# abmoRobotics/isaac_rover_orbit

Hardware: AMD Instinct MI355X
Metric: env-steps/sec AAURoverEnv-v0 @ num_envs=4096; 1/2/4/8 MI355X (higher is better)
Workload: dtype f32

## Files before the change

isaac_rover_orbit_amd/csrc/rover_diag.inc:

```
#pragma once
#if defined(RV_K1_STAMP) || defined(RV_K1_LITE)
__device__ unsigned long long *g_k1_stamps;
#endif
#ifdef RV_K1_LITE
__device__ __forceinline__ void k1_lite(int slot)
{
    if ((threadIdx.x & 255) == 0) {
        unsigned long long t;
        asm volatile("s_memtime %0\n\ts_waitcnt lgkmcnt(0)" : "=s"(t)::"memory");
        g_k1_stamps[(size_t)blockIdx.x * 64 + (threadIdx.x >> 8) * 32 + slot] = t;
    }
}
#define K1_LITE(k) k1_lite(k)
#endif
#ifdef RV_K1_LITE_FINE
#define K1_LITE_F(k) k1_lite(k)
#endif
#ifdef RV_K1_STAMP
__device__ __forceinline__ void k1_stamp(int slot)
{
    if (threadIdx.x == 0) {
        unsigned long long t;
        asm volatile("s_waitcnt vmcnt(0) lgkmcnt(0)\n\ts_memtime %0\n\ts_waitcnt lgkmcnt(0)" : "=s"(t)::"memory");
        g_k1_stamps[(size_t)blockIdx.x * 32 + slot] = t;
    }
}
#define K1_STAMP(k) k1_stamp(k)
#endif
```

isaac_rover_orbit_amd/csrc/rover_kernels.hip:

```cpp
#include <hip/hip_runtime.h>
#include <vector>

#include <cmath>
#include <cstdio>
#include <cstring>
#include <new>
#include <type_traits>

#include <dlfcn.h>

#include "../../include/rover_hip.h"
#include "../../include/rover_debug.h"
#include "rover_model.hpp"
#include "rover_internal.hpp"

namespace {

struct StepConsts {
    float h, inv_h, inv_m, inv_I[3];
    float steer_hkp, steer_den_inv, steer_i_over_h, steer_dv_max;
    float wheel_den_inv, wheel_h_over_i, lt_motor;
    float bogie_keep[3], b_winv[3];
    float bogie_gq[3];
};
__host__ __device__ inline void make_step_consts(float h, StepConsts &k)
{
    constexpr float INERTIA_B[3] = RV_INERTIA_B_INIT;
    constexpr float BOGIE_INERTIA[3] = RV_BOGIE_INERTIA_INIT;
    constexpr float SUBTREE_MASS[3] = RV_SUBTREE_MASS_INIT;
    k.h = h;
    k.inv_h = 1.0f / h;
    k.inv_m = 1.0f / RV_M_TOTAL;
    for (int i = 0; i < 3; ++i) k.inv_I[i] = 1.0f / INERTIA_B[i];
    k.steer_hkp = h * RV_STEER_KP;
    k.steer_den_inv = 1.0f / (RV_STEER_INERTIA + h * RV_STEER_KD + h * h * RV_STEER_KP);
    k.steer_i_over_h = RV_STEER_INERTIA / h;
    k.steer_dv_max = RV_STEER_EFFORT * h / RV_STEER_INERTIA;
    k.wheel_den_inv = 1.0f / (RV_WHEEL_INERTIA + h * RV_WHEEL_KD + h * h * RV_WHEEL_KP);
    k.wheel_h_over_i = h / RV_WHEEL_INERTIA;
    k.lt_motor = RV_WHEEL_EFFORT * h / RV_WHEEL_CONTACT_RADIUS;
    for (int j = 0; j < 3; ++j) {
        k.bogie_keep[j] = 1.0f / (1.0f + h * RV_BOGIE_DAMPING / BOGIE_INERTIA[j]);
        k.b_winv[j] = 1.0f / BOGIE_INERTIA[j];
        k.bogie_gq[j] = (-(SUBTREE_MASS[j] * RV_GRAVITY) * h) * k.b_winv[j];
    }
}

struct RvParams {
    rover_config cfg;
    StepConsts K;
    const float *height;
    const float *lookup;
    const float *obstacle;
    const uint8_t *safe_mask;
    const float *spawns;
    int H, W, n_spawns;
    float res, min_x, min_y;
    int n, env_id_offset;
    uint32_t spawn_a, spawn_b;
    int rays, obs_w;
    int tile_dim;
    int tile_pitch;
    const int16_t *height_q;
    float q_scale;
    int chunk_cells;
    float *scan_desc;
    float inv_res, x_max, y_max, inv_nx;
    int cpr_log;
    int wq, pq;
    int tile_bufs;
    uint32_t step_tag;
    unsigned *log_counter;
    int xcd_rows;
    int nt_obs;
};

__device__ __forceinline__ float clampf(float x, float lo, float hi) { return x < lo ? lo : (x > hi ? hi : x); }
__device__ __forceinline__ float clamp_med3(float x, float lo, float hi) { return __builtin_amdgcn_fmed3f(x, lo, hi); }
__device__ __forceinline__ float dot3(const float *a, const float *b) { return a[0] * b[0] + a[1] * b[1] + a[2] * b[2]; }
__device__ __forceinline__ void cross3(const float *a, const float *b, float *o)
{
    o[0] = a[1] * b[2] - a[2] * b[1];
    o[1] = a[2] * b[0] - a[0] * b[2];
    o[2] = a[0] * b[1] - a[1] * b[0];
}
__device__ __forceinline__ float sign_torch(float x) { return (float)((x > 0.0f) - (x < 0.0f)); }
__device__ __forceinline__ void quat_to_mat(const float *q, float R[3][3])
{
    const float w = q[0], x = q[1], y = q[2], z = q[3];
    R[0][0] = 1.0f - 2.0f * (y * y + z * z);
    R[0][1] = 2.0f * (x * y - w * z);
    R[0][2] = 2.0f * (x * z + w * y);
    R[1][0] = 2.0f * (x * y + w * z);
    R[1][1] = 1.0f - 2.0f * (x * x + z * z);
    R[1][2] = 2.0f * (y * z - w * x);
    R[2][0] = 2.0f * (x * z - w * y);
    R[2][1] = 2.0f * (y * z + w * x);
    R[2][2] = 1.0f - 2.0f * (x * x + y * y);
}
__device__ __forceinline__ void mat_vec(const float R[3][3], const float *v, float *o)
{
    o[0] = R[0][0] * v[0] + R[0][1] * v[1] + R[0][2] * v[2];
    o[1] = R[1][0] * v[0] + R[1][1] * v[1] + R[1][2] * v[2];
    o[2] = R[2][0] * v[0] + R[2][1] * v[1] + R[2][2] * v[2];
}

__device__ __forceinline__ void mat_tvec(const float R[3][3], const float *v, float *o)
{
    o[0] = R[0][0] * v[0] + R[1][0] * v[1] + R[2][0] * v[2];
    o[1] = R[0][1] * v[0] + R[1][1] * v[1] + R[2][1] * v[2];
    o[2] = R[0][2] * v[0] + R[1][2] * v[1] + R[2][2] * v[2];
}
__device__ __forceinline__ float wdot3x(const float *a, const float *b, const float *w) { return a[0] * b[0] * w[0] + a[1] * b[1] * w[1] + a[2] * b[2] * w[2]; }
__device__ __forceinline__ float wdot3(const float *a, const float *w) { return a[0] * a[0] * w[0] + a[1] * a[1] * w[1] + a[2] * a[2] * w[2]; }


__device__ __forceinline__ void rv_sincosf(float x, float *s, float *c)
{
    const float k = floorf(x * 0.63661977236758134f + 0.5f);
    float r = x - k * 1.5703125f;
    r = r - k * 4.837512969970703125e-4f;
    r = r - k * 7.54978995489188e-8f;
    const int q = ((int)k) & 3;
    const float z = r * r;
    const float sp = r + r * z * (-1.6666654611e-1f + z * (8.3321608736e-3f + z * (-1.9515295891e-4f)));
    const float cp = 1.0f - 0.5f * z + z * z * (4.166664568298827e-2f + z * (-1.388731625493765e-3f + z * 2.443315711809948e-5f));
    const float ss = (q & 1) ? cp : sp;
// ... 773 lines not shown
            link_body_forces(lf3[i], Fb);
#pragma unroll
            for (int b = 0; b < 7; ++b) F[b * 3 + i] = Fb[b];
        }
    }
    chassis_integrate(h, R, v, w, com_w, S + ROVER_POS, S + ROVER_QUAT, S + ROVER_LINVEL, S + ROVER_ANGVEL);
#pragma unroll
    for (int j = 0; j < 3; ++j) bogie_integrate(h, bq[j], bd[j], S[ROVER_BOGIE_Q + j], S[ROVER_BOGIE_QD + j]);
}

struct GroupLane {
    float pos[3], quat[4], linvel[3], angvel[3];
    float R[3][3], com_off[3];
    float bq, bqd, sq, sqd, wq, wqd, lam;
    float steer_t, wheel_t;
    float P[3], ax[3], b_winv, bogie_keep;
    float bogie_gq;
    SubConsts sub;
    float lp[3];
    ArmConsts arm;
    f2 minv0, minv1;
    bool steerable, wheel_active, role_b;
};

__device__ __forceinline__ float dpp_ror8(float x) { return __int_as_float(__builtin_amdgcn_update_dpp(0, __float_as_int(x), 0x128, 0xF, 0xF, true)); }
__device__ __forceinline__ void cross_role_sum3(float &a, float &b, float &c)
{
    asm volatile(
        "s_nop 1\n\t"
        "v_add_f32_dpp %0, %0, %0 row_ror:8 row_mask:0xf bank_mask:0xf bound_ctrl:1\n\t"
        "v_add_f32_dpp %1, %1, %1 row_ror:8 row_mask:0xf bank_mask:0xf bound_ctrl:1\n\t"
        "v_add_f32_dpp %2, %2, %2 row_ror:8 row_mask:0xf bank_mask:0xf bound_ctrl:1"
        : "+v"(a), "+v"(b), "+v"(c));
}
__device__ __forceinline__ void slot_sum4(float &a0, float &a1, float &a2, float &a3)
{
    asm volatile(
        "s_nop 1\n\t"
        "v_add_f32_dpp %0, %0, %0 quad_perm:[1,0,3,2] row_mask:0xf bank_mask:0xf bound_ctrl:1\n\t"
        "v_add_f32_dpp %1, %1, %1 quad_perm:[1,0,3,2] row_mask:0xf bank_mask:0xf bound_ctrl:1\n\t"
        "v_add_f32_dpp %2, %2, %2 quad_perm:[1,0,3,2] row_mask:0xf bank_mask:0xf bound_ctrl:1\n\t"
        "v_add_f32_dpp %3, %3, %3 quad_perm:[1,0,3,2] row_mask:0xf bank_mask:0xf bound_ctrl:1\n\t"
        "v_add_f32_dpp %0, %0, %0 quad_perm:[2,3,0,1] row_mask:0xf bank_mask:0xf bound_ctrl:1\n\t"
        "v_add_f32_dpp %1, %1, %1 quad_perm:[2,3,0,1] row_mask:0xf bank_mask:0xf bound_ctrl:1\n\t"
        "v_add_f32_dpp %2, %2, %2 quad_perm:[2,3,0,1] row_mask:0xf bank_mask:0x3 bound_ctrl:1\n\t"
        "v_add_f32_dpp %3, %3, %3 quad_perm:[2,3,0,1] row_mask:0xf bank_mask:0x3 bound_ctrl:1\n\t"
        "v_add_f32_dpp %0, %0, %0 row_half_mirror row_mask:0xf bank_mask:0xf bound_ctrl:1\n\t"
        "v_add_f32_dpp %1, %1, %1 row_half_mirror row_mask:0xf bank_mask:0xf bound_ctrl:1\n\t"
        "v_add_f32_dpp %2, %2, %2 row_half_mirror row_mask:0xf bank_mask:0x3 bound_ctrl:1\n\t"
        "v_add_f32_dpp %3, %3, %3 row_half_mirror row_mask:0xf bank_mask:0x3 bound_ctrl:1"
        : "+v"(a0), "+v"(a1), "+v"(a2), "+v"(a3));
}

#if defined(RV_K1_STAMP) || defined(RV_K1_LITE)
#include "rover_diag.inc"
#endif
#ifndef K1_STAMP
#define K1_STAMP(k) do { } while (0)
#endif
#ifndef K1_LITE
#define K1_LITE(k) do { } while (0)
#endif
#ifndef K1_LITE_F
#define K1_LITE_F(k) do { } while (0)
#endif
__device__ __forceinline__ void solver_iteration_generic(const StepConsts &K, Contact &ct, const RoleRows &rr, f2 *V, float mu)
{
    float un, ut, us;
    role_partials(rr, V, un, ut, us);
    cross_role_sum3(un, ut, us);
    float dn, dt, ds;
    impulse_update(K, ct, mu, un, ut, us, dn, dt, ds);
    f2 o[2];
    role_outputs(rr, dn, dt, ds, o);
    float a0 = o[0].x, a1 = o[0].y, a2 = o[1].x, a3 = o[1].y;
    slot_sum4(a0, a1, a2, a3);
    V[0] += (f2){a0, a1};
    V[1] += (f2){a2, a3};
}

#define RV_DPP_FULL " row_mask:0xf bank_mask:0xf bound_ctrl:1\n\t"
#define RV_DPP_LANES_A " row_mask:0xf bank_mask:0x3 bound_ctrl:1\n\t"
#define RV_BC_LO " op_sel_hi:[1,0,1]\n\t"
#define RV_BC_HI " op_sel:[0,1,0] op_sel_hi:[1,1,1]\n\t"
#define RV_SOLVER_HALF(LN_IN, LN_OUT, LT_IN, LT_OUT, LS_IN, LS_OUT, FILLER)                                            \
    "v_pk_fma_f32 v[240:241], %[jn0], %[v0], %[cn]\n\t"                                                              \
    "v_pk_fma_f32 v[242:243], %[jts0], %[v0], %[cts]" RV_BC_LO                                                       \
    "v_pk_fma_f32 v[240:241], %[jn1], %[v1], v[240:241]\n\t"                                                         \
    "v_pk_fma_f32 v[242:243], %[jts1], %[v0], v[242:243]" RV_BC_HI                                                   \
    "v_add_f32 v240, v240, v241\n\t"                      \
    "v_pk_fma_f32 v[242:243], %[jts2], %[v1], v[242:243]" RV_BC_LO                                                   \
    "v_pk_fma_f32 v[242:243], %[jts3], %[v1], v[242:243]" RV_BC_HI                                                   \
    "v_add_f32_dpp v240, v240, v240 row_ror:8" RV_DPP_FULL    \
    "v_fma_f32 v245, -v240, %[mn], " LN_IN "\n\t"                                                                    \
    "v_add_f32_dpp v242, v242, v242 row_ror:8" RV_DPP_FULL    \
    "v_add_f32_dpp v243, v243, v243 row_ror:8" RV_DPP_FULL    \
    "v_max_f32 " LN_OUT ", 0, v245\n\t"                     \
    "v_sub_f32 v246, " LN_OUT ", " LN_IN "\n\t"             \
    "v_mul_f32 v245, %[mu], " LN_OUT "\n\t"                 \
    "v_pk_mul_f32 v[252:253], %[mn0], v[246:247] op_sel_hi:[1,0]\n\t"                                                \
    "v_fmac_f32 v242, %[ant], v246\n\t"                     \
    "v_pk_mul_f32 v[254:255], %[mn1], v[246:247] op_sel_hi:[1,0]\n\t"                                                \
    "v_min_f32 v247, %[ltm], v245\n\t"                      \
    "v_fmac_f32 v243, %[ans], v246\n\t"                     \
    "v_fma_f32 v244, -v242, %[mt], " LT_IN "\n\t"                                                                    \
    "v_med3_f32 " LT_OUT ", v244, -v247, v247\n\t"          \
    "v_sub_f32 v248, " LT_OUT ", " LT_IN "\n\t"             \
    "v_fmac_f32 v243, %[ats], v248\n\t"                     \
    "v_pk_fma_f32 v[252:253], %[mt0], v[248:249], v[252:253] op_sel_hi:[1,0,1]\n\t"                                  \
    "v_fma_f32 v244, -v243, %[ms], " LS_IN "\n\t"                                                                    \
    "v_pk_fma_f32 v[254:255], %[mt1], v[248:249], v[254:255] op_sel_hi:[1,0,1]\n\t"                                  \
    "v_med3_f32 " LS_OUT ", v244, -v245, v245\n\t"          \
    "v_sub_f32 v250, " LS_OUT ", " LS_IN "\n\t"             \
    "v_pk_fma_f32 v[252:253], %[ms0], v[250:251], v[252:253] op_sel_hi:[1,0,1]\n\t"                                  \
    "v_pk_fma_f32 v[254:255], %[ms1], v[250:251], v[254:255] op_sel_hi:[1,0,1]\n\t"                                  \
    FILLER                                                                                                             \
    "v_add_f32_dpp v252, v252, v252 quad_perm:[1,0,3,2]" RV_DPP_FULL                                                   \
// ... 257 lines not shown
{
    const float cbx = S[ROVER_CMD_B], cby = S[ROVER_CMD_B + 1];
    float *o = obs + (size_t)e * p.obs_w;
    o[0] = S[ROVER_ACTION];
    o[1] = S[ROVER_ACTION + 1];
    o[2] = sqrtf(cbx * cbx + cby * cby) * p.cfg.obs_scale_distance;
    o[3] = rv_atan2f(cby, cbx) * p.cfg.obs_scale_heading;
}

struct ScanWindow {
    float px, py, pz, cy, sy;
    int i_lo, j_lo, th, tw4;
    int interior;
};
__device__ __forceinline__ ScanWindow scan_window(const RvParams &p, const float *pos, const float *quat)
{
    const rover_config &c = p.cfg;
    ScanWindow w;
    const float qw = quat[0], qx = quat[1], qy = quat[2], qz = quat[3];
    const float a = 1.0f - 2.0f * (qy * qy + qz * qz);
    const float b = 2.0f * (qw * qz + qx * qy);
    const float inv = 1.0f / sqrtf(a * a + b * b);
    w.px = pos[0]; w.py = pos[1]; w.pz = pos[2];
    w.cy = a * inv;
    w.sy = b * inv;
    const float inv_res = p.inv_res;
    const float hx = 0.5f * c.scan_size_x, hy = 0.5f * c.scan_size_y;
    const float ex = fabsf(w.cy) * hx + fabsf(w.sy) * hy, ey = fabsf(w.sy) * hx + fabsf(w.cy) * hy;
    int j_lo = (int)floorf((w.px - ex - p.min_x) * inv_res) - 1;
    int i_lo = (int)floorf((w.py - ey - p.min_y) * inv_res) - 1;
    int j_hi = (int)floorf((w.px + ex - p.min_x) * inv_res) + 2;
    int i_hi = (int)floorf((w.py + ey - p.min_y) * inv_res) + 2;
    j_lo = max(0, min(j_lo, p.W - 1)); j_hi = max(0, min(j_hi, p.W - 1));
    i_lo = max(0, min(i_lo, p.H - 1)); i_hi = max(0, min(i_hi, p.H - 1));
    const int cc = p.chunk_cells, sh = (cc == 8) ? 3 : 2;
    j_lo &= ~(cc - 1);
    w.i_lo = i_lo;
    w.j_lo = j_lo;
    w.th = min(i_hi - i_lo + 1, p.tile_dim);
    w.tw4 = min(min((j_hi - j_lo + cc) >> sh, p.tile_pitch >> sh), (p.W - j_lo + cc - 1) >> sh);
    const float m = 2.0f * p.res;
    w.interior = (w.px - ex > p.min_x + m) && (w.px + ex < p.x_max - m) && (w.py - ey > p.min_y + m) &&
                 (w.py + ey < p.y_max - m) && (i_hi - i_lo + 1 <= p.tile_dim) && (((j_hi - j_lo + cc) >> sh) <= (p.tile_pitch >> sh));
    return w;
}
__device__ __forceinline__ void write_scan_desc(const RvParams &p, const float *pos, const float *quat, int e)
{
    const ScanWindow w = scan_window(p, pos, quat);
    float4 *d = reinterpret_cast<float4 *>(p.scan_desc + (size_t)e * 8);
    d[0] = make_float4(w.px, w.py, w.pz, w.cy);
    d[1] = make_float4(w.sy, __int_as_float(w.i_lo), __int_as_float(w.j_lo), __int_as_float(w.th | (w.interior << 15) | (w.tw4 << 16)));
}

__device__ __forceinline__ float wave_sum(float x)
{
#pragma unroll
    for (int m = 32; m >= 1; m >>= 1) x += __shfl_xor(x, m, 64);
    return x;
}

template <int PHASE>
__device__ __forceinline__ void step_lane_body(const RvParams &p, float *__restrict__ state, const float *__restrict__ action,
                                               float *__restrict__ obs, float *__restrict__ reward, uint8_t *__restrict__ terminated,
                                               uint8_t *__restrict__ truncated, float *__restrict__ force, float *__restrict__ log_partial,
                                               const uint8_t *__restrict__ reset_mask)
{
    const int e_raw = blockIdx.x * 64 + threadIdx.x;
    const bool active = e_raw < p.n;
    const int e = active ? e_raw : p.n - 1;
    const int N = p.n;
    const rover_config &c = p.cfg;

    float S[ROVER_STATE_WORDS];
    float F[ROVER_NUM_BODIES * 3];
    if (PHASE == 2) {
#pragma unroll
        for (int i = 0; i < ROVER_STATE_WORDS; ++i) S[i] = state[(size_t)i * N + e];
#pragma unroll
        for (int i = 0; i < ROVER_NUM_BODIES * 3; ++i) F[i] = force[(size_t)i * N + e];
    } else {
#pragma unroll
        for (int i = 0; i < ROVER_TARGET_W; ++i) S[i] = state[(size_t)i * N + e];
#pragma unroll
        for (int i = ROVER_ACTION; i < ROVER_ACTION + 2; ++i) S[i] = state[(size_t)i * N + e];
#pragma unroll
        for (int i = ROVER_LAMBDA_N; i < ROVER_LAMBDA_N + 6; ++i) S[i] = state[(size_t)i * N + e];

        S[ROVER_PREV_ACTION] = S[ROVER_ACTION];
        S[ROVER_PREV_ACTION + 1] = S[ROVER_ACTION + 1];
        const float2 a = reinterpret_cast<const float2 *>(action)[e];
        S[ROVER_ACTION] = a.x;
        S[ROVER_ACTION + 1] = a.y;
        float steer_m[4], wheel_m[6];
        {
            float processed[2], steer[4], wheel[6];
            ackermann_one(c, S + ROVER_ACTION, processed, steer, wheel);
            steer_m[0] = steer[0]; steer_m[1] = steer[3]; steer_m[2] = steer[1]; steer_m[3] = steer[2];
            wheel_m[0] = wheel[1]; wheel_m[1] = wheel[5]; wheel_m[2] = wheel[0];
            wheel_m[3] = wheel[4]; wheel_m[4] = wheel[2]; wheel_m[5] = wheel[3];
        }

        const StepConsts &K = p.K;
        for (int s = 0; s < c.decimation - 1; ++s) physics_substep<false>(p, K, S, steer_m, wheel_m, nullptr);
        if (c.decimation > 0) {
            physics_substep<true>(p, K, S, steer_m, wheel_m, F);
        } else {
// ... 552 lines not shown
                const int r = private_ray_index(m, lane);
                if (r < p.rays) row[r] = o;
            }
        }
    }
}

template <bool TRI>
__device__ __forceinline__ void scan_single_tile_wave(const RvParams &p, int16_t *tile, int lane, int n_env, int e_base,
                                                      const PrivateWindows &w, float *__restrict__ out, int row_stride, int col0,
                                                      const float2 *__restrict__ ray_xy)
{
    if (n_env <= 0) return;
    private_issue(p, w, 0, tile, lane);
    f2 oxy[PRIVATE_ROUNDS];
#pragma unroll
    for (int m = 0; m < PRIVATE_ROUNDS; ++m) {
        const float2 v = ray_xy[m * 64 + lane];
        oxy[m] = (f2){v.x, v.y};
    }
#pragma unroll
    for (int j = 0; j < 4; ++j) {
        if (j < n_env) {
            asm volatile("s_waitcnt vmcnt(0)" ::: "memory");
            __builtin_amdgcn_wave_barrier();
            private_cast<TRI>(p, w, j, tile, lane, e_base, out, row_stride, col0, oxy, ray_xy);
            if (j + 1 < n_env) {
                asm volatile("s_waitcnt lgkmcnt(0)" ::: "memory");
                private_issue(p, w, j + 1, tile, lane);
            }
        }
    }
}

__device__ __forceinline__ void windows_to_lds(float *win, const ScanWindow &sw, int lane)
{
    if ((lane & 15) == 0) {
        float4 *d = reinterpret_cast<float4 *>(win + (lane >> 4) * 8);
        d[0] = make_float4(sw.px, sw.py, sw.pz, sw.cy);
        d[1] = make_float4(sw.sy, __int_as_float(sw.i_lo), __int_as_float(sw.j_lo), __int_as_float(sw.th | (sw.interior << 15) | (sw.tw4 << 16)));
    }
}
__device__ __forceinline__ void windows_from_lds(const float *win, PrivateWindows &w)
{
#pragma unroll
    for (int j = 0; j < 4; ++j) {
        const float4 d0 = reinterpret_cast<const float4 *>(win + j * 8)[0], d1 = reinterpret_cast<const float4 *>(win + j * 8)[1];
        auto uni = [](float v) { return __int_as_float(__builtin_amdgcn_readfirstlane(__float_as_int(v))); };
        w.px[j] = uni(d0.x); w.py[j] = uni(d0.y); w.pz[j] = uni(d0.z); w.cy[j] = uni(d0.w); w.sy[j] = uni(d1.x);
        w.i_lo[j] = __builtin_amdgcn_readfirstlane(__float_as_int(d1.y)); w.j_lo[j] = __builtin_amdgcn_readfirstlane(__float_as_int(d1.z));
        w.pk[j] = __builtin_amdgcn_readfirstlane(__float_as_int(d1.w));
    }
}
constexpr int RV_HAND = 448;
__device__ __forceinline__ float *fused_win(float *lds, const RvParams &p, int wv)
{
    return reinterpret_cast<float *>(reinterpret_cast<int16_t *>(lds) + (size_t)8 * p.tile_dim * p.tile_pitch) + wv * 64;
}
__device__ __forceinline__ float *fused_link(float *lds, const RvParams &p, int wv) { return fused_win(lds, p, 0) + 256 + wv * RV_HAND; }
template <bool TRI>
__device__ __forceinline__ void scan_copy_wave(const RvParams &p, const float *__restrict__ state, float *lds, int partner, int lane,
                                               float *__restrict__ obs, const float2 *__restrict__ ray_xy)
{
    const int tile_cells = p.tile_dim * p.tile_pitch;
    int16_t *tile0 = reinterpret_cast<int16_t *>(lds) + (size_t)(2 * partner) * tile_cells, *tile1 = tile0 + tile_cells;
    const float *win = fused_win(lds, p, partner);
    const int e_base = (int)(blockIdx.x * 4 + partner) * 4;
    const int n_env = max(0, min(4, p.n - e_base));
    PrivateWindows w;
    f2 oxy[PRIVATE_ROUNDS];
#pragma unroll
    for (int m = 0; m < PRIVATE_ROUNDS; ++m) {
        const float2 v = ray_xy[m * 64 + lane];
        oxy[m] = (f2){v.x, v.y};
    }
    {
        const int e = min(e_base + (lane >> 4), p.n - 1);
        const uint32_t count = __float_as_uint(state[(size_t)ROVER_RESET_COUNT * p.n + e]);
        ResetOutcome ro;
        reset_draw(p, (uint32_t)(p.env_id_offset + e), count, nullptr, ro);
        if ((lane & 15) == 0) {
            float4 *d = reinterpret_cast<float4 *>(fused_link(lds, p, partner) + 256 + (lane >> 4) * 12);
            d[0] = make_float4(ro.px, ro.py, ro.pz, ro.qw);
            d[1] = make_float4(ro.qz, ro.tx, ro.ty, ro.tz);
            d[2] = make_float4(ro.heading_cmd, 0.0f, 0.0f, 0.0f);
        }
    }
    {
        __syncthreads();
        const float *lk = fused_link(lds, p, partner);
        const SlotConst sc = d_SLOT[lane & 7];
        const bool role_b = (lane & 8) != 0;
        const float *pe = lk + (lane >> 4) * 12;
        const float R[3][3] = {{pe[0], pe[1], pe[2]}, {pe[3], pe[4], pe[5]}, {pe[6], pe[7], pe[8]}};
        const float pos[3] = {pe[9], pe[10], pe[11]};
        const float P[3] = {sc.P[0], sc.P[1], sc.P[2]}, ax[3] = {sc.ax[0], sc.ax[1], sc.ax[2]};
        float lp[3];
#pragma unroll
        for (int i = 0; i < 3; ++i) lp[i] = role_b ? sc.lp[1][i] : sc.lp[0][i];
        const float bq = lk[64 + lane];
        float bsc[2];
        bogie_sincos(bq, &bsc[0], &bsc[1]);
        const LinkSample ls = link_point_fetch(p, R, pos, P, ax, bq, lp, bsc);
        const float wbp[3] = {sc.wb[0], sc.wb[1], sc.wb[2]};
        const LinkSample ws = link_point_fetch(p, R, pos, P, ax, bq, wbp, bsc);
        float f3[3];
        link_point_eval(ls, p.inv_res, f3);
        const_cast<float *>(lk)[320 + lane] = f3[0];
        const_cast<float *>(lk)[384 + lane] = f3[1];
        const_cast<float *>(lk)[128 + lane] = f3[2];
        const_cast<float *>(lk)[192 + lane] = link_sample_obstacle(ws);
    }
    K1_LITE(0);
    __syncthreads();
    K1_LITE(1);
    {
        float *lk = const_cast<float *>(fused_link(lds, p, partner));
        const float4 d = reinterpret_cast<const float4 *>(lk + 48 + (lane >> 4) * 4)[0];
        const float4 q = reinterpret_cast<const float4 *>(lk + 304 + (lane >> 4) * 4)[0];
        const float pf[3] = {d.x, d.y, d.z}, qf[4] = {q.x, q.y, q.z, q.w};
        const ScanWindow sw = scan_window(p, pf, qf);
        private_windows(sw, w);
        if (n_env > 0) private_issue(p, w, 0, tile0, lane);
        float flag = 0.0f;
        for (int spin = 0; spin < (1 << 20); ++spin) {
            flag = *(volatile __attribute__((address_space(3))) float *)(__attribute__((address_space(3))) float *)(lk + 48 + (lane >> 4) * 4 + 3);
            if (__builtin_amdgcn_ballot_w64(flag == 0.0f) == 0ull) break;
            __builtin_amdgcn_s_sleep(1);
        }
        K1_LITE(2);
        const bool resets = flag == 2.0f;
        const unsigned long long rmask = __builtin_amdgcn_ballot_w64(resets);
        if (__builtin_expect(rmask != 0ull, 0)) {
            float pr[3] = {pf[0], pf[1], pf[2]}, qr[4] = {qf[0], qf[1], qf[2], qf[3]};
            if (resets) {
                const float4 *o = reinterpret_cast<const float4 *>(lk + 256 + (lane >> 4) * 12);
                const float4 o0 = o[0], o1 = o[1];
                pr[0] = o0.x; pr[1] = o0.y; pr[2] = o0.z;
                qr[0] = o0.w; qr[1] = 0.0f; qr[2] = 0.0f; qr[3] = o1.x;
            }
            const ScanWindow swr = scan_window(p, pr, qr);
            private_windows(swr, w);
            uniform_windows(w);
            windows_to_lds(const_cast<float *>(win), swr, lane);
            if (n_env > 0 && (rmask & 0x1ull)) { asm volatile("s_waitcnt vmcnt(0)" ::: "memory"); private_issue(p, w, 0, tile0, lane); }
        } else {
            windows_to_lds(const_cast<float *>(win), sw, lane);
        }
        if ((lane & 15) == 0)
            *(volatile __attribute__((address_space(3))) float *)(__attribute__((address_space(3))) float *)(lk + 48 + (lane >> 4) * 4 + 3) = 3.0f;
    }
    K1_LITE(3);
    asm volatile("s_waitcnt vmcnt(0)" ::: "memory");
    K1_LITE(4);
    if (n_env > 0) private_cast<TRI>(p, w, 0, tile0, lane, e_base, obs, p.obs_w, 4, oxy, ray_xy);
    K1_LITE(5);
    asm volatile("s_waitcnt lgkmcnt(0)" ::: "memory");
    K1_LITE(6);
    K1_LITE(7);
    if (n_env > 2) private_issue(p, w, 2, tile0, lane);
    K1_LITE(8);
    asm volatile("s_waitcnt vmcnt(0)" ::: "memory");
    K1_LITE(9);
    K1_LITE(10);
    K1_LITE(11);
    if (n_env > 2) private_cast<TRI>(p, w, 2, tile0, lane, e_base, obs, p.obs_w, 4, oxy, ray_xy);
    K1_LITE(12);
    K1_LITE(13);
    K1_LITE(14);
    K1_LITE(15);
}

enum StepForm { TWO_LAUNCH, COPY_WAVES, SINGLE_TILE };
template <StepForm FORM, bool TRI, bool BEGIN_ONLY = false>
__device__ __forceinline__ void step_group_body(const RvParams &p, float *__restrict__ state, const float *__restrict__ action,
                                                float *__restrict__ obs, float *__restrict__ reward, uint8_t *__restrict__ terminated,
                                                uint8_t *__restrict__ truncated, float *__restrict__ force,
                                                float *__restrict__ log_partial, float *lds, const float2 *__restrict__ ray_xy)
{
    const int lane = threadIdx.x & 63;
    const int wave = blockIdx.x * (RV_K1G_THREADS / 64) + (threadIdx.x >> 6);
    const int e_raw = wave * 4 + (lane >> 4);
    const bool active = e_raw < p.n;
    const int e = active ? e_raw : p.n - 1;
    const int N = p.n;
    const rover_config &c = p.cfg;
    const SlotConst sc = d_SLOT[lane & 7];
    const GroupIds id = group_ids(lane, sc);
    K1_STAMP(0);
    K1_LITE(0);

    const StepConsts &K = p.K;
    GroupLane g;
    group_load(state, N, e, id, sc, K, g, p.cfg.mass_model);
    float act[2], prev[2];
    prev[0] = state[(size_t)(ROVER_ACTION + 0) * N + e];
    prev[1] = state[(size_t)(ROVER_ACTION + 1) * N + e];
    const float2 a = reinterpret_cast<const float2 *>(action)[e];
    act[0] = a.x;
    act[1] = a.y;
    float S[ROVER_STATE_WORDS];
    {
        float processed[2], steer[4], rim[6];
        ackermann_core(c, act, processed, steer, rim);
        const float steer_m[4] = {steer[0], steer[3], steer[1], steer[2]};
        const float rim_m[6] = {rim[1], rim[5], rim[0], rim[4], rim[2], rim[3]};
        float st = steer_m[0], rv = rim_m[0];
#pragma unroll
        for (int i = 1; i < 4; ++i) st = (id.si == i) ? steer_m[i] : st;
#pragma unroll
        for (int i = 1; i < 6; ++i) rv = (id.k == i) ? rim_m[i] : rv;
        g.steer_t = st;
        g.wheel_t = rv / c.wheel_radius;
    }
    float Fw[6] = {0.0f, 0.0f, 0.0f, 0.0f, 0.0f, 0.0f};
    f2 oxy[PRIVATE_ROUNDS];
    K1_STAMP(1);
    for (int s = 0; s < c.decimation - 1; ++s) physics_substep_group<false>(p, K, g, nullptr, s);
#pragma unroll
    for (int i = ROVER_TARGET_W; i < ROVER_ACTION; ++i) S[i] = state[(size_t)i * N + e];
#pragma unroll
    for (int i = ROVER_TIME_LEFT; i < ROVER_LAMBDA_N; ++i) S[i] = state[(size_t)i * N + e];
    S[ROVER_RESET_COUNT] = state[(size_t)ROVER_RESET_COUNT * N + e];
    if constexpr (FORM == COPY_WAVES) {
        const int wv = __builtin_amdgcn_readfirstlane((int)(threadIdx.x >> 6));
        float *lk = fused_link(lds, p, wv);
        if ((lane & 15) == 0) {
            float4 *d = reinterpret_cast<float4 *>(lk + (lane >> 4) * 12);
            d[0] = make_float4(g.R[0][0], g.R[0][1], g.R[0][2], g.R[1][0]);
            d[1] = make_float4(g.R[1][1], g.R[1][2], g.R[2][0], g.R[2][1]);
            d[2] = make_float4(g.R[2][2], g.pos[0], g.pos[1], g.pos[2]);
        }
        lk[64 + lane] = g.bq;
        __syncthreads();
        if (c.decimation > 0) physics_substep_group<true, true>(p, K, g, Fw, c.decimation - 1);
    } else {
        if (c.decimation > 0) physics_substep_group<true>(p, K, g, Fw, c.decimation - 1);
    }
    K1_STAMP(20);
    K1_LITE(1);
    if constexpr (FORM == COPY_WAVES) {
        const int wv = __builtin_amdgcn_readfirstlane((int)(threadIdx.x >> 6));
        float *lk = fused_link(lds, p, wv);
        if ((lane & 15) == 0) {
            float4 *d = reinterpret_cast<float4 *>(lk + 48 + (lane >> 4) * 4);
            float4 *q = reinterpret_cast<float4 *>(lk + 304 + (lane >> 4) * 4);
            d[0] = make_float4(g.pos[0], g.pos[1], g.pos[2], 0.0f);
            q[0] = make_float4(g.quat[0], g.quat[1], g.quat[2], g.quat[3]);
        }
        __syncthreads();
        if (c.decimation > 0) {
            const int wv = __builtin_amdgcn_readfirstlane((int)(threadIdx.x >> 6));
            const float *lk = fused_link(lds, p, wv);
            Fw[3] = lk[320 + lane]; Fw[4] = lk[384 + lane]; Fw[5] = lk[128 + lane];
            if (!(lk[192 + lane] > RV_OBSTACLE_EPS)) { Fw[0] = 0.0f; Fw[1] = 0.0f; Fw[2] = 0.0f; }
        }
    }
    if (!id.wheel_active) { Fw[0] = 0.0f; Fw[1] = 0.0f; Fw[2] = 0.0f; Fw[3] = 0.0f; Fw[4] = 0.0f; Fw[5] = 0.0f; }
    float F[ROVER_NUM_BODIES * 3];
#pragma unroll
    for (int i = 0; i < ROVER_NUM_BODIES * 3; ++i) F[i] = 0.0f;
    const bool any_force = __ballot(Fw[0] != 0.0f || Fw[1] != 0.0f || Fw[2] != 0.0f || Fw[5] != 0.0f) != 0ull;
    if (__builtin_expect(any_force, 0)) {
        constexpr int BODY_SLOT[6] = {1, 3, 0, 2, 4, 5};
        const int base = lane & ~15;
#pragma unroll
        for (int b = 0; b < 6; ++b)
#pragma unroll
            for (int i = 0; i < 3; ++i) F[(7 + b) * 3 + i] = __shfl(Fw[i], base + BODY_SLOT[b], 64);
#pragma unroll
        for (int i = 0; i < 3; ++i) {
            float lf[6][2], Fb[7];
#pragma unroll
            for (int sl = 0; sl < 6; ++sl) {
                lf[sl][0] = __shfl(Fw[3 + i], base + sl, 64);
                lf[sl][1] = __shfl(Fw[3 + i], base + 8 + sl, 64);
            }
            link_body_forces(lf, Fb);
#pragma unroll
            for (int b = 0; b < 7; ++b) F[b * 3 + i] = Fb[b];
        }
    }
    int coll_known = -1;
    if constexpr (FORM == COPY_WAVES) {
        const int wv = __builtin_amdgcn_readfirstlane((int)(threadIdx.x >> 6));
        const bool coll = any_force ? collision_measure(F) > 1.0f : false;
        coll_known = coll ? 1 : 0;
        bool term_e[ROVER_NUM_TERM];
        mdp_terminations(c, S + ROVER_CMD_B, __float_as_int(S[ROVER_EP_LEN]) + 1, coll, term_e);
        if ((lane & 15) == 0)
            *(volatile __attribute__((address_space(3))) float *)(__attribute__((address_space(3))) float *)(fused_link(lds, p, wv) + 48 + (lane >> 4) * 4 + 3) =
                (term_e[0] | term_e[1] | term_e[2] | term_e[3]) ? 2.0f : 1.0f;
        K1_LITE(2);
#pragma unroll
        for (int m = 0; m < PRIVATE_ROUNDS; ++m) {
            const float2 v = ray_xy[m * 64 + lane];
            oxy[m] = (f2){v.x, v.y};
        }
    }
    K1_LITE_F(11);
    if (active) group_store(state, N, e, id, g, lane);
    K1_LITE_F(12);
    if (force && active && id.owner) {
#pragma unroll
        for (int i = 0; i < 3; ++i) *soa_word(force, id.body * 3 + i, N, e) = Fw[i];
    }
    if (force && active && (lane & 15) < 7) {
#pragma unroll
        for (int i = 0; i < 3; ++i) {
            float fb = F[i];
#pragma unroll
            for (int b = 1; b < 7; ++b) fb = ((lane & 15) == b) ? F[b * 3 + i] : fb;
            *soa_word(force, (lane & 15) * 3 + i, N, e) = fb;
        }
    }
    K1_STAMP(23);
    K1_LITE_F(13);

#pragma unroll
    for (int i = 0; i < 3; ++i) S[ROVER_POS + i] = g.pos[i];
#pragma unroll
    for (int i = 0; i < 4; ++i) S[ROVER_QUAT + i] = g.quat[i];
    S[ROVER_ACTION] = act[0]; S[ROVER_ACTION + 1] = act[1];
    S[ROVER_PREV_ACTION] = prev[0]; S[ROVER_PREV_ACTION + 1] = prev[1];
#pragma unroll
    for (int i = ROVER_LINVEL; i < ROVER_TARGET_W; ++i) S[i] = 0.0f;
#pragma unroll
    for (int i = ROVER_LAMBDA_N; i < ROVER_LAMBDA_N + 6; ++i) S[i] = 0.0f;

    const int ep_len = __float_as_int(S[ROVER_EP_LEN]) + 1;
    S[ROVER_EP_LEN] = __int_as_float(ep_len);
    float rew[ROVER_NUM_REW];
    bool term[ROVER_NUM_TERM];
    mdp_terms_one(c, S + ROVER_CMD_B, S + ROVER_ACTION, S + ROVER_PREV_ACTION, ep_len, F, rew, term, !any_force, coll_known);
    K1_STAMP(24);
    K1_LITE_F(14);
    const bool time_out = term[0];
    const bool term_any = term[1] | term[2] | term[3];
    const float step_dt = c.sim_dt * (float)c.decimation;
    float total = 0.0f;
#pragma unroll
    for (int i = 0; i < ROVER_NUM_REW; ++i) {
// ... 73 lines not shown
            p.log_counter[0] = 1u;
            p.log_counter[1] = p.step_tag;
        }
    }
    if (active) {
        const int r = lane & 15;
        {
            float *o = obs + (size_t)e * p.obs_w;
            const float cbx = S[ROVER_CMD_B], cby = S[ROVER_CMD_B + 1];
            const float head[4] = {S[ROVER_ACTION], S[ROVER_ACTION + 1], sqrtf(cbx * cbx + cby * cby) * p.cfg.obs_scale_distance,
                                   rv_atan2f(cby, cbx) * p.cfg.obs_scale_heading};
            const float x = pick_by_lane<1, 4, 0, 4>(r, head, head[0]);
            if (r < 4) o[r] = x;
        }
        if (FORM == TWO_LAUNCH && r == 0) write_scan_desc(p, S + ROVER_POS, S + ROVER_QUAT, e);
        if (do_reset) store_rows_by_lane<ROVER_POS, 7, ROVER_POS>(state, N, e, r, S);
        static_assert(ROVER_LAMBDA_N - ROVER_TARGET_W == 26, "manager words 39..64");
        store_rows_by_lane<ROVER_TARGET_W, 16, ROVER_TARGET_W>(state, N, e, r, S);
        store_rows_by_lane<ROVER_TARGET_W + 16, 10, ROVER_TARGET_W + 16>(state, N, e, r, S);
        if (r == 0) {
            state[(size_t)ROVER_RESET_COUNT * N + e] = S[ROVER_RESET_COUNT];
            reward[e] = total;
            terminated[e] = term_any ? 1 : 0;
            truncated[e] = time_out ? 1 : 0;
        }
    }
    K1_STAMP(25);
    if constexpr (FORM == SINGLE_TILE) {
        const int tile_cells = p.tile_dim * p.tile_pitch;
        const int wv = __builtin_amdgcn_readfirstlane((int)(threadIdx.x >> 6));
        int16_t *tile = reinterpret_cast<int16_t *>(lds) + (size_t)wv * tile_cells;
        PrivateWindows pw;
        private_windows(scan_window(p, S + ROVER_POS, S + ROVER_QUAT), pw);
        scan_single_tile_wave<TRI>(p, tile, lane, max(0, min(4, p.n - wave * 4)), wave * 4, pw, obs, p.obs_w, 4, ray_xy);
        K1_STAMP(26);
    }
    if constexpr (FORM == COPY_WAVES) {
        const int tile_cells = p.tile_dim * p.tile_pitch;
        const int wv = __builtin_amdgcn_readfirstlane((int)(threadIdx.x >> 6));
        int16_t *tile0 = reinterpret_cast<int16_t *>(lds) + (size_t)(2 * wv) * tile_cells, *tile1 = tile0 + tile_cells;
        float *win = fused_win(lds, p, wv);
        const int n_scan = max(0, min(4, p.n - wave * 4));
        const int e_base = wave * 4;
        K1_LITE(3);
        K1_LITE(4);
        PrivateWindows pw;
        {
            const float *lk = fused_link(lds, p, wv);
            for (int spin = 0; spin < (1 << 20); ++spin) {
                const float f = *(volatile __attribute__((address_space(3))) float *)(__attribute__((address_space(3))) float *)(const_cast<float *>(lk) + 48 + (lane >> 4) * 4 + 3);
                if (__builtin_amdgcn_ballot_w64(f != 3.0f) == 0ull) break;
                __builtin_amdgcn_s_sleep(1);
            }
        }
        windows_from_lds(win, pw);
        K1_LITE(5);
        K1_STAMP(27);
        if (n_scan > 1) {
            private_issue(p, pw, 1, tile1, lane);
            asm volatile("s_waitcnt vmcnt(0)" ::: "memory");
            private_cast<TRI>(p, pw, 1, tile1, lane, e_base, obs, p.obs_w, 4, oxy, ray_xy);
            asm volatile("s_waitcnt lgkmcnt(0)" ::: "memory");
        }
        K1_STAMP(28);
        K1_LITE(6);
        K1_LITE(7);
        if (n_scan > 3) {
            private_issue(p, pw, 3, tile1, lane);
            K1_LITE(8);
            asm volatile("s_waitcnt vmcnt(0)" ::: "memory");
            K1_STAMP(29);
            K1_LITE(9);
            private_cast<TRI>(p, pw, 3, tile1, lane, e_base, obs, p.obs_w, 4, oxy, ray_xy);
        }
        K1_STAMP(26);
        K1_LITE(10);
    }
}
__global__ __launch_bounds__(RV_K1G_THREADS) void rover_step_begin_kernel(RvParams p, float *__restrict__ state,
                                                                          const float *__restrict__ action, float *__restrict__ reward,
                                                                          uint8_t *__restrict__ terminated, uint8_t *__restrict__ truncated,
                                                                          float *__restrict__ force)
{
    step_group_body<TWO_LAUNCH, false, true>(p, state, action, nullptr, reward, terminated, truncated, force, nullptr, nullptr, nullptr);
}
__global__ __launch_bounds__(RV_K1G_THREADS) void rover_step_kernel_group(RvParams p, float *__restrict__ state,
                                                              const float *__restrict__ action, float *__restrict__ obs,
                                                              float *__restrict__ reward, uint8_t *__restrict__ terminated,
                                                              uint8_t *__restrict__ truncated, float *__restrict__ force,
                                                              float *__restrict__ log_partial)
{
    step_group_body<TWO_LAUNCH, false>(p, state, action, obs, reward, terminated, truncated, force, log_partial, nullptr, nullptr);
}
template <bool TRI>
__global__ __launch_bounds__(2 * RV_K1G_THREADS) RV_FUSED_ATTR void rover_step_scan_kernel(
    RvParams p, float *__restrict__ state, const float *__restrict__ action, float *__restrict__ obs, float *__restrict__ reward,
    uint8_t *__restrict__ terminated, uint8_t *__restrict__ truncated, float *__restrict__ force, float *__restrict__ log_partial,
    const float2 *__restrict__ ray_xy)
{
    extern __shared__ __align__(16) float lds[];
    const int wv = __builtin_amdgcn_readfirstlane((int)(threadIdx.x >> 6));
    if (wv < RV_K1G_THREADS / 64) {
        step_group_body<COPY_WAVES, TRI>(p, state, action, obs, reward, terminated, truncated, force, log_partial, lds, ray_xy);
    } else {
        scan_copy_wave<TRI>(p, state, lds, wv - RV_K1G_THREADS / 64, (int)(threadIdx.x & 63), obs, ray_xy);
    }
}

__global__ __launch_bounds__(RV_K1G_THREADS) void rover_physics_kernel_group(RvParams p, float *__restrict__ state,
                                                                             const float *steer_t, const float *wheel_t,
                                                                             int substeps, float *force)
{
    const int lane = threadIdx.x & 63;
// ... 1173 lines not shown
    for (int i = 0; i < 3; ++i) HIP_TRY(hipEventCreate(&ev[i]));
    double acc = 0.0;
    for (int r = 0; r < reps; ++r) {
        HIP_TRY(hipEventRecord(ev[0], st));
        HIP_TRY(hipEventRecord(ev[1], st));
        HIP_TRY(hipEventRecord(ev[2], st));
        HIP_TRY(hipEventSynchronize(ev[2]));
        float a = 0.0f, b = 0.0f;
        HIP_TRY(hipEventElapsedTime(&a, ev[0], ev[1]));
        HIP_TRY(hipEventElapsedTime(&b, ev[1], ev[2]));
        acc += 0.5 * ((double)a + (double)b);
    }
    for (int i = 0; i < 3; ++i) HIP_TRY(hipEventDestroy(ev[i]));
    *ms = (float)(acc / reps);
    return ROVER_OK;
}

int rover_mdp_terms(rover_sim *sim, int32_t n, const float *cmd_b, const float *action, const float *prev_action,
                    const int32_t *ep_len, const float *force, float *obs_distance, float *obs_angle, float *rew,
                    uint8_t *term, void *stream)
{
    if (!sim || n <= 0 || !cmd_b || !action || !prev_action || !ep_len || !force || !obs_distance || !obs_angle || !rew || !term)
        return fail(ROVER_ERR_INVALID, "bad argument");
    DeviceGuard guard(sim->device);
    hipLaunchKernelGGL(rover_mdp_terms_kernel, dim3((n + 127) / 128), dim3(128), 0, static_cast<hipStream_t>(stream), sim->p.cfg,
                       n, cmd_b, action, prev_action, ep_len, force, obs_distance, obs_angle, rew, term);
    HIP_TRY(hipGetLastError());
    return ROVER_OK;
}

int rover_ackermann(rover_sim *sim, int32_t n, const float *raw, float *processed, float *steer, float *wheel, void *stream)
{
    if (!sim || !raw || !processed || !steer || !wheel || n <= 0) return fail(ROVER_ERR_INVALID, "bad argument");
    DeviceGuard guard(sim->device);
    hipLaunchKernelGGL(rover_ackermann_kernel, dim3((n + 255) / 256), dim3(256), 0, static_cast<hipStream_t>(stream),
                       sim->p.cfg, n, raw, processed, steer, wheel);
    HIP_TRY(hipGetLastError());
    return ROVER_OK;
}

int rover_height_scan(rover_sim *sim, float *scan, void *stream)
{
    if (int rc = ready(sim)) return rc;
    if (!scan) return fail(ROVER_ERR_INVALID, "scan is NULL");
    DeviceGuard guard(sim->device);
    const RvParams &p = sim->p;
    launch_scan<0>(sim, p.n, static_cast<hipStream_t>(stream), scan, p.rays, 0, nullptr, 0, nullptr);
    HIP_TRY(hipGetLastError());
    return ROVER_OK;
}

int rover_debug_set_fused(rover_sim *sim, int fused)
{
    if (!sim || fused < -1 || fused > 2) return ROVER_ERR_INVALID;
    sim->fused = fused;
    return ROVER_OK;
}
#if defined(RV_K1_STAMP) || defined(RV_K1_LITE)
int rover_debug_set_k1_stamps(void *buf)
{
    return hipMemcpyToSymbol(HIP_SYMBOL(g_k1_stamps), &buf, sizeof(buf)) == hipSuccess ? ROVER_OK : ROVER_ERR_HIP;
}
#endif

int rover_physics(rover_sim *sim, const float *steer_target, const float *wheel_target, int32_t substeps, float *force,
                  void *stream)
{
    if (int rc = ready(sim)) return rc;
    if (!steer_target || !wheel_target || substeps < 0) return fail(ROVER_ERR_INVALID, "bad argument");
    DeviceGuard guard(sim->device);
    if (sim->group_mapping)
        hipLaunchKernelGGL(rover_physics_kernel_group, dim3((sim->p.n + RV_K1G_ENVS - 1) / RV_K1G_ENVS), dim3(RV_K1G_THREADS), 0, static_cast<hipStream_t>(stream),
                           sim->p, sim->state, steer_target, wheel_target, substeps, force);
    else
        hipLaunchKernelGGL(rover_physics_kernel, dim3((sim->p.n + 63) / 64), dim3(64), 0, static_cast<hipStream_t>(stream),
                           sim->p, sim->state, steer_target, wheel_target, substeps, force);
    HIP_TRY(hipGetLastError());
    return ROVER_OK;
}

int rover_model_constants(float *out, int32_t cap)
{
    const float com[3] = RV_COM_B_INIT, inertia[3] = RV_INERTIA_B_INIT, wheel[6][3] = RV_WHEEL_B_INIT;
    const float pivot[3][3] = RV_BOGIE_PIVOT_INIT, axis[3][3] = RV_BOGIE_AXIS_INIT, binertia[3] = RV_BOGIE_INERTIA_INIT;
    float t[160];
    int n = 0;
    t[n++] = RV_M_TOTAL;
    for (int i = 0; i < 3; ++i) t[n++] = com[i];
    for (int i = 0; i < 3; ++i) t[n++] = inertia[i];
    for (int k = 0; k < 6; ++k) for (int i = 0; i < 3; ++i) t[n++] = wheel[k][i];
    for (int k = 0; k < 3; ++k) for (int i = 0; i < 3; ++i) t[n++] = pivot[k][i];
    for (int k = 0; k < 3; ++k) for (int i = 0; i < 3; ++i) t[n++] = axis[k][i];
    for (int k = 0; k < 3; ++k) t[n++] = binertia[k];
    t[n++] = RV_WHEEL_CONTACT_RADIUS;
    t[n++] = RV_STEER_INERTIA; t[n++] = RV_STEER_KP; t[n++] = RV_STEER_KD; t[n++] = RV_STEER_EFFORT; t[n++] = RV_STEER_VLIM;
    t[n++] = RV_WHEEL_INERTIA; t[n++] = RV_WHEEL_KP; t[n++] = RV_WHEEL_KD; t[n++] = RV_WHEEL_EFFORT; t[n++] = RV_WHEEL_VLIM;
    t[n++] = RV_BOGIE_QLIM; t[n++] = RV_BOGIE_DAMPING; t[n++] = RV_BAUMGARTE; t[n++] = RV_MAX_DEPENETRATION_VEL;
    t[n++] = RV_MAX_LINEAR_VEL; t[n++] = RV_GRAVITY; t[n++] = RV_OBSTACLE_EPS; t[n++] = RV_WARM_START; t[n++] = RV_STEER_QLIM;
    {
        const float lp[6][2][3] = RV_LINK_POINT_INIT;
        for (int sl = 0; sl < 6; ++sl) for (int r = 0; r < 2; ++r) for (int i = 0; i < 3; ++i) t[n++] = lp[sl][r][i];
        for (int sl = 0; sl < 6; ++sl) for (int r = 0; r < 2; ++r) for (int i = 0; i < 3; ++i)
            if (d_SLOT_host_lp(sl, r, i) != lp[sl][r][i]) return -1;
        t[n++] = RV_LINK_STIFFNESS;
    }
    {
        const float sm[3] = RV_SUBTREE_MASS_INIT, scom[3][3] = RV_SUBTREE_COM_INIT;
        for (int j = 0; j < 3; ++j) t[n++] = sm[j];
        for (int j = 0; j < 3; ++j) for (int i = 0; i < 3; ++i) {
            if (d_SLOT_host_sc(j, i) != scom[j][i]) return -1;
// ... 14 lines not shown
```

Baseline: 102.1 million.

## Prefetch height-scan tiles early from predicted pose before physics sync

Before the block barrier, the scan wave predicts each env's next pose from the pre-step position and velocities, builds a padded scan window, and issues its tile loads early. If the real post-physics window fits inside the prefetched one, the tile is reused and the second load and its wait are skipped, with a kept-mask passed through LDS to the copy wave. The goal is to hide global load latency of the height tiles behind the physics phase. It adds velocity stores to LDS, extra fences and a larger LDS hand-off region, and loads are wasted when the prediction misses.

```diff
diff --git a/isaac_rover_orbit_amd/csrc/rover_diag.inc b/isaac_rover_orbit_amd/csrc/rover_diag.inc
--- a/isaac_rover_orbit_amd/csrc/rover_diag.inc
+++ b/isaac_rover_orbit_amd/csrc/rover_diag.inc
@@ -27,3 +27,14 @@
 }
 #define K1_STAMP(k) k1_stamp(k)
 #endif
+#ifdef RV_STAGE_COUNTER
+__device__ unsigned *g_stage_count;
+__device__ __forceinline__ void stage_count(unsigned kept, int staged)
+{
+    if ((threadIdx.x & 63) == 0 && g_stage_count) {
+        atomicAdd(g_stage_count, (unsigned)__builtin_popcount(kept));
+        atomicAdd(g_stage_count + 1, (unsigned)staged);
+    }
+}
+#define RV_STAGE_COUNT(kept, staged) stage_count(kept, staged)
+#endif
diff --git a/isaac_rover_orbit_amd/csrc/rover_kernels.hip b/isaac_rover_orbit_amd/csrc/rover_kernels.hip
--- a/isaac_rover_orbit_amd/csrc/rover_kernels.hip
+++ b/isaac_rover_orbit_amd/csrc/rover_kernels.hip
@@ -73,6 +73,7 @@
     unsigned *log_counter;
     int xcd_rows;
     int nt_obs;
+    int stage_mode;
 };
 
 __device__ __forceinline__ float clampf(float x, float lo, float hi) { return x < lo ? lo : (x > hi ? hi : x); }
@@ -952,7 +953,7 @@
         : "+v"(a0), "+v"(a1), "+v"(a2), "+v"(a3));
 }
 
-#if defined(RV_K1_STAMP) || defined(RV_K1_LITE)
+#if defined(RV_K1_STAMP) || defined(RV_K1_LITE) || defined(RV_STAGE_COUNTER)
 #include "rover_diag.inc"
 #endif
 #ifndef K1_STAMP
@@ -963,6 +964,9 @@
 #endif
 #ifndef K1_LITE_F
 #define K1_LITE_F(k) do { } while (0)
+#endif
+#ifndef RV_STAGE_COUNT
+#define RV_STAGE_COUNT(kept, staged) do { } while (0)
 #endif
 __device__ __forceinline__ void solver_iteration_generic(const StepConsts &K, Contact &ct, const RoleRows &rr, f2 *V, float mu)
 {
@@ -1326,6 +1330,34 @@
     d[1] = make_float4(w.sy, __int_as_float(w.i_lo), __int_as_float(w.j_lo), __int_as_float(w.th | (w.interior << 15) | (w.tw4 << 16)));
 }
 
+__device__ __forceinline__ ScanWindow staged_window(const RvParams &p, float px, float py, float a, float b)
+{
+    const rover_config &c = p.cfg;
+    ScanWindow w;
+    const float inv = 1.0f / sqrtf(a * a + b * b);
+    w.px = px; w.py = py; w.pz = 0.0f;
+    w.cy = a * inv;
+    w.sy = b * inv;
+    const float inv_res = p.inv_res;
+    const float hx = 0.5f * c.scan_size_x, hy = 0.5f * c.scan_size_y;
+    const float ex = fabsf(w.cy) * hx + fabsf(w.sy) * hy, ey = fabsf(w.sy) * hx + fabsf(w.cy) * hy;
+    int j_lo = (int)floorf((w.px - ex - p.min_x) * inv_res) - 2;
+    int i_lo = (int)floorf((w.py - ey - p.min_y) * inv_res) - 2;
+    int j_hi = (int)floorf((w.px + ex - p.min_x) * inv_res) + 3;
+    int i_hi = (int)floorf((w.py + ey - p.min_y) * inv_res) + 3;
+    i_lo += max(i_hi - i_lo + 1 - p.tile_dim, 0) >> 1;
+    j_lo = max(0, min(j_lo, p.W - 1)); j_hi = max(0, min(j_hi, p.W - 1));
+    i_lo = max(0, min(i_lo, p.H - 1)); i_hi = max(0, min(i_hi, p.H - 1));
+    const int cc = p.chunk_cells, sh = (cc == 8) ? 3 : 2;
+    j_lo &= ~(cc - 1);
+    w.i_lo = i_lo;
+    w.j_lo = j_lo;
+    w.th = min(i_hi - i_lo + 1, p.tile_dim);
+    w.tw4 = min(min((j_hi - j_lo + cc) >> sh, p.tile_pitch >> sh), (p.W - j_lo + cc - 1) >> sh);
+    w.interior = 0;
+    return w;
+}
+
 __device__ __forceinline__ float wave_sum(float x)
 {
 #pragma unroll
@@ -1984,7 +2016,8 @@
         w.pk[j] = __builtin_amdgcn_readfirstlane(__float_as_int(d1.w));
     }
 }
-constexpr int RV_HAND = 448;
+constexpr int RV_HAND = 480;
+constexpr int RV_WIN_KEPT = 32;
 __device__ __forceinline__ float *fused_win(float *lds, const RvParams &p, int wv)
 {
     return reinterpret_cast<float *>(reinterpret_cast<int16_t *>(lds) + (size_t)8 * p.tile_dim * p.tile_pitch) + wv * 64;
@@ -2044,22 +2077,58 @@
         const_cast<float *>(lk)[192 + lane] = link_sample_obstacle(ws);
     }
     K1_LITE(0);
+    const bool early = p.stage_mode != 1;
+    ScanWindow st;
+    st.i_lo = 0; st.j_lo = 0; st.th = 0; st.tw4 = 0;
+    if (early) {
+        const float *lk = fused_link(lds, p, partner);
+        const float *pe = lk + (lane >> 4) * 12;
+        const float4 lv = reinterpret_cast<const float4 *>(lk + 448 + (lane >> 4) * 8)[0];
+        const float4 av = reinterpret_cast<const float4 *>(lk + 448 + (lane >> 4) * 8)[1];
+        const float h = p.K.h;
+        const float a = pe[0] + h * (av.y * pe[6] - av.z * pe[3]);
+        const float b = pe[3] + h * (av.z * pe[0] - av.x * pe[6]);
+        st = staged_window(p, pe[9] + h * lv.x, pe[10] + h * lv.y, a, b);
+        PrivateWindows ws;
+        private_windows(st, ws);
+        if (n_env > 0) private_issue(p, ws, 0, tile0, lane);
+        if (n_env > 1) private_issue(p, ws, 1, tile1, lane);
+    }
+    K1_LITE(13);
     __syncthreads();
     K1_LITE(1);
     {
         float *lk = const_cast<float *>(fused_link(lds, p, partner));
+        if (early) asm volatile("s_waitcnt vmcnt(0)" ::: "memory");
         const float4 d = reinterpret_cast<const float4 *>(lk + 48 + (lane >> 4) * 4)[0];
         const float4 q = reinterpret_cast<const float4 *>(lk + 304 + (lane >> 4) * 4)[0];
         const float pf[3] = {d.x, d.y, d.z}, qf[4] = {q.x, q.y, q.z, q.w};
         const ScanWindow sw = scan_window(p, pf, qf);
-        private_windows(sw, w);
-        if (n_env > 0) private_issue(p, w, 0, tile0, lane);
+        const int cc = p.chunk_cells;
+        auto covers = [&](const ScanWindow &t) {
+            return st.i_lo <= t.i_lo && t.i_lo + t.th <= st.i_lo + st.th && st.j_lo <= t.j_lo && t.j_lo + t.tw4 * cc <= st.j_lo + st.tw4 * cc;
+        };
+        auto final_window = [&](const ScanWindow &t, bool k) {
+            ScanWindow f = t;
+            f.i_lo = k ? st.i_lo : t.i_lo; f.j_lo = k ? st.j_lo : t.j_lo; f.th = k ? st.th : t.th; f.tw4 = k ? st.tw4 : t.tw4;
+            return f;
+        };
+        auto kept_bits = [](bool k) {
+            const unsigned long long m = __builtin_amdgcn_ballot_w64(k);
+            return (unsigned)(m & 1ull) | ((unsigned)(m >> 15) & 2u);
+        };
+        bool keep = early && p.stage_mode != 2 && (lane >> 4) < min(n_env, 2) && covers(sw);
+        unsigned kept = kept_bits(keep);
+        ScanWindow fin = final_window(sw, keep);
+        private_windows(fin, w);
+        if (n_env > 0 && !(kept & 1u)) private_issue(p, w, 0, tile0, lane);
         float flag = 0.0f;
         for (int spin = 0; spin < (1 << 20); ++spin) {
             flag = *(volatile __attribute__((address_space(3))) float *)(__attribute__((address_space(3))) float *)(lk + 48 + (lane >> 4) * 4 + 3);
             if (__builtin_amdgcn_ballot_w64(flag == 0.0f) == 0ull) break;
             __builtin_amdgcn_s_sleep(1);
         }
+        __builtin_amdgcn_fence(__ATOMIC_ACQUIRE, "workgroup");
         K1_LITE(2);
         const bool resets = flag == 2.0f;
         const unsigned long long rmask = __builtin_amdgcn_ballot_w64(resets);
@@ -2072,18 +2141,22 @@
                 qr[0] = o0.w; qr[1] = 0.0f; qr[2] = 0.0f; qr[3] = o1.x;
             }
             const ScanWindow swr = scan_window(p, pr, qr);
-            private_windows(swr, w);
+            keep = keep && !resets;
+            kept = kept_bits(keep);
+            fin = final_window(swr, keep);
+            private_windows(fin, w);
             uniform_windows(w);
-            windows_to_lds(const_cast<float *>(win), swr, lane);
             if (n_env > 0 && (rmask & 0x1ull)) { asm volatile("s_waitcnt vmcnt(0)" ::: "memory"); private_issue(p, w, 0, tile0, lane); }
-        } else {
-            windows_to_lds(const_cast<float *>(win), sw, lane);
-        }
+        }
+        RV_STAGE_COUNT(kept, min(n_env, 2));
+        windows_to_lds(const_cast<float *>(win), fin, lane);
+        if (lane == 0) const_cast<float *>(win)[RV_WIN_KEPT] = __uint_as_float(kept);
+        __builtin_amdgcn_fence(__ATOMIC_RELEASE, "workgroup");
         if ((lane & 15) == 0)
             *(volatile __attribute__((address_space(3))) float *)(__attribute__((address_space(3))) float *)(lk + 48 + (lane >> 4) * 4 + 3) = 3.0f;
-    }
-    K1_LITE(3);
-    asm volatile("s_waitcnt vmcnt(0)" ::: "memory");
+        K1_LITE(3);
+        if (!(kept & 1u)) asm volatile("s_waitcnt vmcnt(0)" ::: "memory");
+    }
     K1_LITE(4);
     if (n_env > 0) private_cast<TRI>(p, w, 0, tile0, lane, e_base, obs, p.obs_w, 4, oxy, ray_xy);
     K1_LITE(5);
@@ -2098,7 +2171,6 @@
     K1_LITE(11);
     if (n_env > 2) private_cast<TRI>(p, w, 2, tile0, lane, e_base, obs, p.obs_w, 4, oxy, ray_xy);
     K1_LITE(12);
-    K1_LITE(13);
     K1_LITE(14);
     K1_LITE(15);
 }
@@ -2162,6 +2234,9 @@
             d[0] = make_float4(g.R[0][0], g.R[0][1], g.R[0][2], g.R[1][0]);
             d[1] = make_float4(g.R[1][1], g.R[1][2], g.R[2][0], g.R[2][1]);
             d[2] = make_float4(g.R[2][2], g.pos[0], g.pos[1], g.pos[2]);
+            float4 *v = reinterpret_cast<float4 *>(lk + 448 + (lane >> 4) * 8);
+            v[0] = make_float4(g.linvel[0], g.linvel[1], g.linvel[2], 0.0f);
+            v[1] = make_float4(g.angvel[0], g.angvel[1], g.angvel[2], 0.0f);
         }
         lk[64 + lane] = g.bq;
         __syncthreads();
@@ -2220,6 +2295,7 @@
         coll_known = coll ? 1 : 0;
         bool term_e[ROVER_NUM_TERM];
         mdp_terminations(c, S + ROVER_CMD_B, __float_as_int(S[ROVER_EP_LEN]) + 1, coll, term_e);
+        __builtin_amdgcn_fence(__ATOMIC_RELEASE, "workgroup");
         if ((lane & 15) == 0)
             *(volatile __attribute__((address_space(3))) float *)(__attribute__((address_space(3))) float *)(fused_link(lds, p, wv) + 48 + (lane >> 4) * 4 + 3) =
                 (term_e[0] | term_e[1] | term_e[2] | term_e[3]) ? 2.0f : 1.0f;
@@ -2399,13 +2475,17 @@
                 if (__builtin_amdgcn_ballot_w64(f != 3.0f) == 0ull) break;
                 __builtin_amdgcn_s_sleep(1);
             }
+            __builtin_amdgcn_fence(__ATOMIC_ACQUIRE, "workgroup");
         }
         windows_from_lds(win, pw);
+        const unsigned kept = (unsigned)__builtin_amdgcn_readfirstlane(__float_as_int(win[RV_WIN_KEPT]));
         K1_LITE(5);
         K1_STAMP(27);
         if (n_scan > 1) {
-            private_issue(p, pw, 1, tile1, lane);
-            asm volatile("s_waitcnt vmcnt(0)" ::: "memory");
+            if (!(kept & 2u)) {
+                private_issue(p, pw, 1, tile1, lane);
+                asm volatile("s_waitcnt vmcnt(0)" ::: "memory");
+            }
             private_cast<TRI>(p, pw, 1, tile1, lane, e_base, obs, p.obs_w, 4, oxy, ray_xy);
             asm volatile("s_waitcnt lgkmcnt(0)" ::: "memory");
         }
@@ -3685,10 +3765,17 @@
 
 int rover_debug_set_fused(rover_sim *sim, int fused)
 {
-    if (!sim || fused < -1 || fused > 2) return ROVER_ERR_INVALID;
-    sim->fused = fused;
+    if (!sim || fused < -1 || fused > 4) return ROVER_ERR_INVALID;
+    sim->fused = fused >= 3 ? 1 : fused;
+    sim->p.stage_mode = fused == 3 ? 1 : fused == 4 ? 2 : 0;
     return ROVER_OK;
 }
+#ifdef RV_STAGE_COUNTER
+int rover_debug_set_stage_counter(void *buf)
+{
+    return hipMemcpyToSymbol(HIP_SYMBOL(g_stage_count), &buf, sizeof(buf)) == hipSuccess ? ROVER_OK : ROVER_ERR_HIP;
+}
+#endif
 #if defined(RV_K1_STAMP) || defined(RV_K1_LITE)
 int rover_debug_set_k1_stamps(void *buf)
 {
```

Result: slower. 95.17 million (-6.8%).
